# tongdaxu/VQ-VAE-from-Gaussian-VAE

Hardware: AMD Instinct MI355X
Metric: images/sec encode+quantize+decode, 256x256, codebook 2^16 (higher is better)
Workload: dtype f32

## Files before the change

### include/gqhip.h

```cpp
#ifndef GQHIP_H_
#define GQHIP_H_

#include <stdint.h>

#ifdef __cplusplus
extern "C" {
#endif

#define GQHIP_ABI_VERSION 8

typedef int64_t gqhip_gnstat_t;
#define GQHIP_GNSTAT_WORDS 8

typedef enum gqhip_status {
  GQHIP_OK = 0,
  GQHIP_ERR_INVALID_ARG = 1,
  GQHIP_ERR_WORKSPACE = 2,
  GQHIP_ERR_LAUNCH = 3,
  GQHIP_ERR_NO_DEVICE = 4
} gqhip_status;

int gqhip_abi_version(void);
const char *gqhip_status_string(int status);
int gqhip_last_hip_error(void);
// ... 73 lines not shown

int fsq_quantize_f32(const float *z, const int32_t *levels_host, int64_t nlev, float *zhat,
                     int32_t *idx, int64_t rows, void *stream);
int fsq_dequant_f32(const int32_t *idx, const int32_t *levels_host, int64_t nlev, float *zhat,
                    int64_t rows, void *stream);

#define GQHIP_LAYOUT_NCHW 0
#define GQHIP_LAYOUT_NHWC 1
int gn_silu_f32(const float *x, const float *gamma, const float *beta,
                const float *pre_bias_or_null, float *y, int64_t B, int64_t C, int64_t HW,
                int64_t groups, double eps, int apply_silu, int layout, gqhip_gnstat_t *stats_ws,
                void *stream);
int add_bias_f32(const float *a, const float *b, const float *bias_or_null, float *y, int64_t B,
                 int64_t C, int64_t HW, int layout, void *stream);

int add_bias_stats_f32(const float *a, const float *b, const float *bias_or_null, float *y, int64_t B,
                       int64_t C, int64_t HW, int64_t groups, gqhip_gnstat_t *stats_out, void *stream);

int gn_apply_f32(const float *x, const float *gamma, const float *beta, float *y, int64_t B, int64_t C,
                 int64_t HW, int64_t groups, double eps, int apply_silu, const gqhip_gnstat_t *stats, void *stream);

int gqhip_checksum_tensors(const void *table_dev, int64_t count, uint64_t *sums_dev, void *stream);

int gqhip_stats_prezeroed(int on);

int conv3x3_cin_small_f32(const float *x, const float *wk, const float *bias_or_null, float *y, int64_t *stats_out_or_null,
                          int64_t B, int64_t H, int64_t W, int64_t Cin, int64_t Cout, int64_t groups_out, void *stream);

int conv3x3_f32(const float *x, const float *gamma_or_null, const float *beta_or_null, const float *pre_bias_or_null,
                const gqhip_gnstat_t *stats_or_null, int64_t groups_in, double eps, int apply_silu, const float *wk,
                const float *bias_or_null, float *y, int64_t B, int64_t H, int64_t W, int64_t Cin, int64_t Cout, void *stream);

int upsample2x_nhwc_f32(const float *x, float *y, int64_t B, int64_t H, int64_t W, int64_t C,
                        void *stream);

int wino_in_nhwc_f32(const float *x, float *V, int64_t B, int64_t H, int64_t W, int64_t C, void *stream);
int wino_out_nhwc_f32(const float *M, float *y, int64_t B, int64_t H, int64_t W, int64_t C, float mscale, void *stream);

int wino_in_nhwc_f16x3(const float *x, void *V3, int64_t B, int64_t H, int64_t W, int64_t C, int tile, float scale,
                       void *stream);
int wino_in_nhwc_f16x2(const float *x, void *V2, int64_t B, int64_t H, int64_t W, int64_t C, int tile, float scale,
                       void *stream);
int wino_gemm_f16x2(const void *V2, const void *Wf, float *M, int64_t P, int64_t tiles, int64_t Cin, int64_t Cout,
                    void *stream);
int conv3x3_gn_f16x3(const float *x, const float *gamma, const float *beta, const float *pre_bias_or_null,
                     const gqhip_gnstat_t *stats_in, int64_t groups_in, double eps, int apply_silu, float scale, const void *Wf,
                     const float *bias_or_null, const float *res_or_null, float *y, gqhip_gnstat_t *stats_out_or_null, int64_t B,
                     int64_t H, int64_t W, int64_t Cin, int64_t Cout, int64_t groups_out, float mscale, void *stream);
int conv1x1_f16x3(const float *x, const float *pre_bias_or_null, const void *Wf, const float *scales_dev_or_null, float scale,
                  float mscale, const float *bias_or_null, const float *res_or_null, float *y, gqhip_gnstat_t *stats_out_or_null, int64_t B, int64_t HW,
                  int64_t Cin, int64_t Cout, int64_t groups_out, void *stream);
int conv1x1_gn_f16x3(const float *x, const float *gamma, const float *beta, const float *pre_bias_or_null,
                     const gqhip_gnstat_t *stats_in, int64_t groups_in, double eps, const void *Wf, float scale, float mscale,
                     const float *bias_or_null, const float *res_or_null, float *y, gqhip_gnstat_t *stats_out_or_null, int64_t B,
                     int64_t HW, int64_t Cin, int64_t Cout, int64_t groups_out, void *stream);
int conv1x1_qkv_split_f16x3(const float *x, const float *gamma_or_null, const float *beta_or_null, const float *pre_bias_or_null,
                            const gqhip_gnstat_t *stats_in_or_null, int64_t groups_in, double eps, const void *Wf, float scale,
                            float mscale, const float *bias_or_null, void *Q3, void *K3, void *V3, float sq, float sv, int64_t B,
                            int64_t L, int64_t C, void *stream);
int conv3x3s2_f16x3(const float *x, const void *Wf, const float *scales_dev_or_null, float scale, float mscale,
                    const float *bias_or_null, float *y, gqhip_gnstat_t *stats_out_or_null, int64_t B, int64_t Hin, int64_t Win,
                    int64_t Cin, int64_t Cout, int64_t groups_out, void *stream);
int upconv2x_f16x3(const float *x, const void *Wf, const float *scales_dev_or_null, float scale, float mscale,
                   const float *bias_or_null, float *y, gqhip_gnstat_t *stats_out_or_null, int64_t B, int64_t H, int64_t W,
                   int64_t Cin, int64_t Cout, int64_t groups_out, void *stream);
int conv3x3_gn_small_f32(const float *x, const float *gamma, const float *beta, const float *pre_bias_or_null,
                         const gqhip_gnstat_t *stats_in, int64_t groups_in, double eps, int apply_silu, const float *w_ohwi,
                         const float *bias_or_null, float *y, int64_t B, int64_t H, int64_t W, int64_t Cin, int64_t Cout,
                         void *stream);
int wino_in_gn_nhwc_f16x3(const float *x, const float *gamma, const float *beta, const float *pre_bias_or_null,
                          const gqhip_gnstat_t *stats, void *V3, int64_t B, int64_t H, int64_t W, int64_t C, int64_t groups,
                          double eps, int apply_silu, int tile, float scale, void *stream);
int wino_in_gn_nhwc_f16x2(const float *x, const float *gamma, const float *beta, const float *pre_bias_or_null,
                          const gqhip_gnstat_t *stats, void *V2, int64_t B, int64_t H, int64_t W, int64_t C, int64_t groups,
                          double eps, int apply_silu, int tile, float scale, void *stream);

int wino4_in_nhwc_f32(const float *x, float *V, int64_t B, int64_t H, int64_t W, int64_t C, void *stream);
int wino4_out_nhwc_f32(const float *M, float *y, int64_t B, int64_t H, int64_t W, int64_t C, float mscale, void *stream);

int wino_out_res_nhwc_f32(const float *M, const float *res, const float *bias_or_null, float *y, gqhip_gnstat_t *stats_out,
                          int64_t B, int64_t H, int64_t W, int64_t C, int64_t groups, int tile, float mscale,
                          void *stream);

int gn_stats_f32(const float *x, const float *pre_bias_or_null, int64_t B, int64_t C, int64_t HW, int64_t groups,
                 gqhip_gnstat_t *stats_out, void *stream);

int wino_in_gn_nhwc_f32(const float *x, const float *gamma, const float *beta, const float *pre_bias_or_null,
                        const gqhip_gnstat_t *stats, float *V, int64_t B, int64_t H, int64_t W, int64_t C,
                        int64_t groups, double eps, int apply_silu, void *stream);
int wino4_in_gn_nhwc_f32(const float *x, const float *gamma, const float *beta, const float *pre_bias_or_null,
                         const gqhip_gnstat_t *stats, float *V, int64_t B, int64_t H, int64_t W, int64_t C,
                         int64_t groups, double eps, int apply_silu, void *stream);

int attn_split_qkv_f16x3(const float *qkv, void *Q3, void *K3, void *V3, int64_t B, int64_t L, int64_t C, float sq, float sv,
                         void *stream);
int attn_softmax_split_f16x3(const float *S, void *P3, int64_t rows, int64_t L, float factor, void *stream);
int f16_scales_from_gn_stats(const gqhip_gnstat_t *stats, int64_t n_bg, double amp, double u_scale, float *scales_out,
                             void *stream);

int gq_index_histogram(const int64_t *idx, int64_t count, int64_t n,
                       int32_t *hist, void *stream);
int gq_indices_to_u16(const int64_t *idx, uint16_t *out, int64_t count,
                      void *stream);
int gq_indices_from_u16(const uint16_t *in, int64_t *idx, int64_t count,
                        void *stream);

int64_t gq_step_record_workspace_bytes(int64_t B, int64_t per_image);
int gq_step_record_f32(const float *x, const float *x_rec, const int64_t *idx, int32_t *rec, int64_t B, int64_t per_image,
                       int64_t n_idx, void *workspace_zeroed, int64_t workspace_bytes, void *stream);

int64_t gq_ssim_workspace_bytes(int64_t B, int64_t C, int64_t H, int64_t W);
int gq_ssim_f32(const float *x, const float *x_rec, int64_t B, int64_t C, int64_t H, int64_t W, int layout, int zero_mean,
                float *ssim_out_or_null, float *msssim_out_or_null, void *workspace_zeroed, int64_t workspace_bytes, void *stream);
int64_t gq_step_record_ssim_workspace_bytes(int64_t B, int64_t C, int64_t H, int64_t W);
int gq_step_record_ssim_f32(const float *x, const float *x_rec, const int64_t *idx, int32_t *rec, int64_t B, int64_t C, int64_t H,
                            int64_t W, int layout, int64_t n_idx, void *workspace_zeroed, int64_t workspace_bytes, void *stream);

int64_t gq_mha_workspace_bytes(int64_t B, int64_t L, int64_t E, int64_t H);
int gq_mha_fwd_f32(const float *qkv, float *out, int64_t B, int64_t L, int64_t E, int64_t H, void *workspace, void *stream);

int gqhip_profile_enable(int on);
int gqhip_profile_reserve(int pairs);
int gqhip_profile_collect(int *launches_host, double *total_ms_host);

int gqhip_debug_enable(int on);
int gqhip_debug_counters(const void *workspace, int64_t *fallback_rows_host,
                         int64_t *reranked_halftiles_host);
int gqhip_debug_grid(const void *workspace, const void *cb_cache_or_null, int64_t *out4_host);
#ifdef __cplusplus
}
#endif
#endif
```

### vq-vae-from-gaussian-vae_amd/csrc/gqhip_unet.hip

```cpp
#include "gqhip.h"

#include <hip/hip_ext.h>
#include <hip/hip_runtime.h>

#include <cstdlib>
#include <cstring>

#include "gqhip_internal.h"
#include "gq_unet_aux.h"
#include "gq_wino_gemm.h"
#include "gq_conv3.h"
#include "gq_conv_f32.h"
#include "gq_attn.h"

using namespace gqhip;

namespace {
thread_local int g_stats_prezeroed = 0;
inline hipError_t stats_zero(void *p, size_t bytes, hipStream_t st) {
  return g_stats_prezeroed ? hipSuccess : hipMemsetAsync(p, 0, bytes, st);
}
}

extern "C" {

int gqhip_stats_prezeroed(int on) {
  g_stats_prezeroed = on != 0;
  return GQHIP_OK;
}

int gn_silu_f32(const float *x, const float *gamma, const float *beta, const float *pre_bias_or_null, float *y,
                int64_t B, int64_t C, int64_t HW, int64_t groups, double eps, int apply_silu, int layout,
                int64_t *stats_ws, void *stream) {
  if (B < 0 || C < 1 || HW < 1 || groups < 1 || C % groups != 0) return GQHIP_ERR_INVALID_ARG;
  if (B == 0) return GQHIP_OK;
  if (!x || !gamma || !beta || !y || !stats_ws) return GQHIP_ERR_INVALID_ARG;
  hipStream_t st = static_cast<hipStream_t>(stream);
  const int64_t bg = B * groups, cpg = C / groups, chunk = cpg * HW;
  if (layout == GQHIP_LAYOUT_NHWC) {
    if (cpg % 4 != 0 || 256 % (C / 4) != 0 || groups > 64) return GQHIP_ERR_INVALID_ARG;
    if (stats_zero(stats_ws, sizeof(int64_t) * kStatWords * bg, st) != hipSuccess) return check_launch();
    const int lanes = (int)(256 / (C / 4));
    int slabs = (int)((HW + (int64_t)lanes * 16 - 1) / ((int64_t)lanes * 16));
    if (slabs > 1024) slabs = 1024;
    if (slabs < 1) slabs = 1;
    hipLaunchKernelGGL(gn_stats_nhwc_kernel, dim3((unsigned)(B * slabs)), dim3(256), 0, st, x, pre_bias_or_null,
                       stats_ws, (int)C, (long)HW, (int)cpg, slabs);
    int rc = check_launch();
    if (rc != GQHIP_OK) return rc;
    return launch(apply_silu ? gn_apply_nhwc_kernel<1> : gn_apply_nhwc_kernel<0>, dim3((unsigned)(B * slabs)), dim3(256), 0, st, x,
                  gamma, beta, y, stats_ws, pre_bias_or_null, (int)C, (long)HW, (int)cpg, eps, slabs);
  }
  if (layout != GQHIP_LAYOUT_NCHW || HW % 4 != 0) return GQHIP_ERR_INVALID_ARG;
  if (stats_zero(stats_ws, sizeof(int64_t) * kStatWords * bg, st) != hipSuccess) return check_launch();
  int slices = (int)((chunk + 4095) / 4096);
  if (slices > 256) slices = 256;
  if (slices < 1) slices = 1;
  hipLaunchKernelGGL(gn_stats_kernel, dim3((unsigned)(bg * slices)), dim3(256), 0, st, x, pre_bias_or_null, stats_ws,
                     (long)chunk, slices, (long)HW, (int)cpg, (int)groups);
  int rc = check_launch();
  if (rc != GQHIP_OK) return rc;
  int segs = (int)((HW + 8191) / 8192);
  if (segs < 1) segs = 1;
  const dim3 grid((unsigned)(B * C * segs));
  return launch(apply_silu ? gn_apply_kernel<1> : gn_apply_kernel<0>, grid, dim3(256), 0, st, x, gamma, beta, y, stats_ws,
                pre_bias_or_null, (int)C, (long)HW, (int)cpg, eps, segs);
}

int add_bias_f32(const float *a, const float *b, const float *bias_or_null, float *y, int64_t B, int64_t C,
                 int64_t HW, int layout, void *stream) {
  if (B < 0 || C < 1 || HW < 1) return GQHIP_ERR_INVALID_ARG;
  if (B == 0) return GQHIP_OK;
  if (!a || !b || !y) return GQHIP_ERR_INVALID_ARG;
  const long total4 = (long)(B * C * HW / 4);
  long blocks = (total4 + 255) / 256;
  if (blocks > 8192) blocks = 8192;
  hipStream_t st = static_cast<hipStream_t>(stream);
  if (layout == GQHIP_LAYOUT_NHWC) {
    if (C % 4 != 0) return GQHIP_ERR_INVALID_ARG;
    hipLaunchKernelGGL(add_bias_nhwc_kernel, dim3((unsigned)blocks), dim3(256), 0, st, a, b, bias_or_null, y, (int)C,
                       total4);
  } else {
    if (layout != GQHIP_LAYOUT_NCHW || HW % 4 != 0) return GQHIP_ERR_INVALID_ARG;
    hipLaunchKernelGGL(add_bias_kernel, dim3((unsigned)blocks), dim3(256), 0, st, a, b, bias_or_null, y, (int)C,
                       (long)HW, total4);
  }
  return check_launch();
}

static int nhwc_slabs(int64_t C, int64_t HW) {
  const int lanes = (int)(256 / (C / 4));
  int slabs = (int)((HW + (int64_t)lanes * 16 - 1) / ((int64_t)lanes * 16));
  if (slabs > 1024) slabs = 1024;
  return slabs < 1 ? 1 : slabs;
}

int add_bias_stats_f32(const float *a, const float *b, const float *bias_or_null, float *y, int64_t B, int64_t C,
                       int64_t HW, int64_t groups, int64_t *stats_out, void *stream) {
  if (B < 0 || C < 1 || HW < 1 || groups < 1 || C % groups != 0) return GQHIP_ERR_INVALID_ARG;
  if (B == 0) return GQHIP_OK;
  if (!a || !b || !y || !stats_out) return GQHIP_ERR_INVALID_ARG;
  const int64_t cpg = C / groups;
  if (cpg % 4 != 0 || 256 % (C / 4) != 0 || groups > 64) return GQHIP_ERR_INVALID_ARG;
  hipStream_t st = static_cast<hipStream_t>(stream);
// ... 444 lines not shown
  cp.H = (int)H; cp.W = (int)W; cp.Cin = (int)Cin; cp.Cout = (int)Cout; cp.cpg = gn ? (int)(Cin / groups_in) : 1; cp.eps = eps;
  const unsigned segs = (unsigned)(B * H * ((W + 31) / 32));
  if (Cin % 64 == 0) {
    const dim3 grid(segs, (unsigned)((Cout + 31) / 32));
    if (gn && apply_silu) hipLaunchKernelGGL((conv3x3_f32_ksplit_kernel<true, 1>), grid, dim3(256), 0, st, cp);
    else if (gn) hipLaunchKernelGGL((conv3x3_f32_ksplit_kernel<true, 0>), grid, dim3(256), 0, st, cp);
    else hipLaunchKernelGGL((conv3x3_f32_ksplit_kernel<false, 0>), grid, dim3(256), 0, st, cp);
    return check_launch();
  }
  if (gn) return GQHIP_ERR_INVALID_ARG;
  switch (Cin) {
    case 8: hipLaunchKernelGGL((conv3x3_f32_nsplit_kernel<8>), dim3(segs), dim3(256), 0, st, cp); break;
    case 16: hipLaunchKernelGGL((conv3x3_f32_nsplit_kernel<16>), dim3(segs), dim3(256), 0, st, cp); break;
    case 32: hipLaunchKernelGGL((conv3x3_f32_nsplit_kernel<32>), dim3(segs), dim3(256), 0, st, cp); break;
    default: return GQHIP_ERR_INVALID_ARG;
  }
  return check_launch();
}

int wino_out_nhwc_f32(const float *M, float *y, int64_t B, int64_t H, int64_t W, int64_t C, float mscale, void *stream) {
  if (B < 0 || H < 2 || W < 2 || H % 2 || W % 2 || C < 4 || C % 4 != 0) return GQHIP_ERR_INVALID_ARG;
  if (B == 0) return GQHIP_OK;
  if (!M || !y) return GQHIP_ERR_INVALID_ARG;
  const long tiles = (long)(B * (H / 2) * (W / 2)), total = tiles * (C / 4);
  long blocks = (total + 255) / 256;
  if (blocks > 16384) blocks = 16384;
  return launch(wino_out_nhwc_kernel, dim3((unsigned)blocks), dim3(256), 0, static_cast<hipStream_t>(stream), M, y,
                (int)H, (int)W, (int)(C / 4), tiles, total, mscale);
}

int wino4_in_nhwc_f32(const float *x, float *V, int64_t B, int64_t H, int64_t W, int64_t C, void *stream) {
  if (B < 0 || H < 4 || W < 4 || H % 4 || W % 4 || C < 4 || C % 4 != 0) return GQHIP_ERR_INVALID_ARG;
  if (B == 0) return GQHIP_OK;
  if (!x || !V) return GQHIP_ERR_INVALID_ARG;
  const long tiles = (long)(B * (H / 4) * (W / 4)), total = tiles * (C / 4);
  long blocks = (total + 255) / 256;
  if (blocks > 16384) blocks = 16384;
  return launch(wino4_in_nhwc_kernel<0>, dim3((unsigned)blocks), dim3(256), 0, static_cast<hipStream_t>(stream), x,
                (void *)V, (int)H, (int)W, (int)(C / 4), tiles, total, 1.0f);
}

int wino4_out_nhwc_f32(const float *M, float *y, int64_t B, int64_t H, int64_t W, int64_t C, float mscale, void *stream) {
  if (B < 0 || H < 4 || W < 4 || H % 4 || W % 4 || C < 4 || C % 4 != 0) return GQHIP_ERR_INVALID_ARG;
  if (B == 0) return GQHIP_OK;
  if (!M || !y) return GQHIP_ERR_INVALID_ARG;
  const long tiles = (long)(B * (H / 4) * (W / 4)), total = tiles * (C / 4);
  long blocks = (total + 255) / 256;
  if (blocks > 16384) blocks = 16384;
  return launch(wino4_out_nhwc_kernel, dim3((unsigned)blocks), dim3(256), 0, static_cast<hipStream_t>(stream), M, y,
                (int)H, (int)W, (int)(C / 4), tiles, total, mscale);
}

int wino_out_res_nhwc_f32(const float *M, const float *res, const float *bias_or_null, float *y, int64_t *stats_out,
                          int64_t B, int64_t H, int64_t W, int64_t C, int64_t groups, int tile, float mscale,
                          void *stream) {
  if ((tile != 2 && tile != 4) || B < 0 || H < tile || W < tile || H % tile || W % tile || C < 4 || C % 4 != 0 ||
      groups < 1 || C % groups != 0)
    return GQHIP_ERR_INVALID_ARG;
  if (B == 0) return GQHIP_OK;
  if (!M || !y || !stats_out) return GQHIP_ERR_INVALID_ARG;
  const int64_t cpg = C / groups;
  if (cpg % 4 != 0 || 256 % (C / 4) != 0 || groups > 64) return GQHIP_ERR_INVALID_ARG;
  hipStream_t st = static_cast<hipStream_t>(stream);
  if (stats_zero(stats_out, sizeof(int64_t) * kStatWords * B * groups, st) != hipSuccess) return check_launch();
  const long tpi = (long)((H / tile) * (W / tile)), tiles = (long)B * tpi;
  const int vw = (tile == 4 && 256 % (C / 2) == 0) ? 2 : 4;
  const int lanes = (int)(256 / (C / vw));
  long slabs = (tpi + (long)lanes * 4 - 1) / ((long)lanes * 4);
  if (slabs > 1024) slabs = 1024;
  if (slabs < 1) slabs = 1;
  const dim3 grid((unsigned)(B * slabs));
  if (tile == 4 && vw == 2)
    hipLaunchKernelGGL((wino_out_res_nhwc_kernel<4, 2>), grid, dim3(256), 0, st, M, res, bias_or_null, y, stats_out, (int)H,
                       (int)W, (int)(C / 2), (int)cpg, tiles, (int)slabs, mscale);
  else if (tile == 4)
    hipLaunchKernelGGL((wino_out_res_nhwc_kernel<4, 4>), grid, dim3(256), 0, st, M, res, bias_or_null, y, stats_out, (int)H,
                       (int)W, (int)(C / 4), (int)cpg, tiles, (int)slabs, mscale);
  else
    hipLaunchKernelGGL((wino_out_res_nhwc_kernel<2, 4>), grid, dim3(256), 0, st, M, res, bias_or_null, y, stats_out, (int)H,
                       (int)W, (int)(C / 4), (int)cpg, tiles, (int)slabs, mscale);
  return check_launch();
}

int attn_split_qkv_f16x3(const float *qkv, void *Q3, void *K3, void *V3, int64_t B, int64_t L, int64_t C, float sq, float sv,
                         void *stream) {
  if (B < 0 || L < 1 || C < 4 || C % 4 != 0 || !(sq > 0.f) || !(sv > 0.f)) return GQHIP_ERR_INVALID_ARG;
  if (B == 0) return GQHIP_OK;
  if (!qkv || !Q3 || !K3 || !V3) return GQHIP_ERR_INVALID_ARG;
  const long total = (long)(B * L * (C / 4));
  long blocks = (total + 255) / 256;
  if (blocks > 16384) blocks = 16384;
  return launch(attn_split_qkv_kernel, dim3((unsigned)blocks), dim3(256), 0, static_cast<hipStream_t>(stream), qkv,
                static_cast<_Float16 *>(Q3), static_cast<_Float16 *>(K3), static_cast<_Float16 *>(V3), (long)L,
                (int)(C / 4), sq, sv, total);
}

int attn_softmax_split_f16x3(const float *S, void *P3, int64_t rows, int64_t L, float factor, void *stream) {
  if (rows < 0 || L < 64 || L % 64 != 0 || L > 4096 || !(factor > 0.f)) return GQHIP_ERR_INVALID_ARG;
  if (rows == 0) return GQHIP_OK;
  if (!S || !P3) return GQHIP_ERR_INVALID_ARG;
  const dim3 grid((unsigned)((rows + 3) / 4));
  hipStream_t st = static_cast<hipStream_t>(stream);
  _Float16 *p = static_cast<_Float16 *>(P3);
#define GQ_SM(N) hipLaunchKernelGGL(attn_softmax_split_kernel<N>, grid, dim3(256), 0, st, S, p, (long)rows, factor)
  switch (L / 64) {
    case 1: GQ_SM(1); break;
    case 4: GQ_SM(4); break;
    case 16: GQ_SM(16); break;
    case 36: GQ_SM(36); break;
    case 64: GQ_SM(64); break;
    default: return GQHIP_ERR_INVALID_ARG;
  }
#undef GQ_SM
  return check_launch();
}

int f16_scales_from_gn_stats(const int64_t *stats, int64_t n_bg, double amp, double u_scale, float *scales_out,
                             void *stream) {
  if (!stats || !scales_out || n_bg < 1 || n_bg > 0x7fffffff || !(amp > 0.0) || !(u_scale > 0.0)) return GQHIP_ERR_INVALID_ARG;
  return launch(f16_scales_from_stats_kernel, dim3(1), dim3(64), 0, static_cast<hipStream_t>(stream), stats, (int)n_bg,
                (float)amp, (float)u_scale, scales_out);
}

int upsample2x_nhwc_f32(const float *x, float *y, int64_t B, int64_t H, int64_t W, int64_t C, void *stream) {
  if (B < 0 || H < 1 || W < 1 || C < 4 || C % 4 != 0) return GQHIP_ERR_INVALID_ARG;
  if (B == 0) return GQHIP_OK;
  if (!x || !y) return GQHIP_ERR_INVALID_ARG;
  const long total = (long)(B * H * W * (C / 4));
  long blocks = (total + 255) / 256;
  if (blocks > 16384) blocks = 16384;
  return launch(upsample2x_nhwc_kernel, dim3((unsigned)blocks), dim3(256), 0, static_cast<hipStream_t>(stream), x,
                y, (int)H, (int)W, (int)(C / 4), total);
}

int gqhip_checksum_tensors(const void *table_dev, int64_t count, uint64_t *sums_dev, void *stream) {
  if (count < 0 || count > 65535) return GQHIP_ERR_INVALID_ARG;
  if (count == 0) return GQHIP_OK;
  if (!table_dev || !sums_dev) return GQHIP_ERR_INVALID_ARG;
  hipStream_t st = static_cast<hipStream_t>(stream);
  if (hipMemsetAsync(sums_dev, 0, sizeof(uint64_t) * count, st) != hipSuccess) return check_launch();
  return launch(checksum_tensors_kernel, dim3((unsigned)count, kChecksumSlices), dim3(256), 0, st,
                static_cast<const ChecksumEntry *>(table_dev), reinterpret_cast<unsigned long long *>(sums_dev));
}

int64_t gq_mha_workspace_bytes(int64_t B, int64_t L, int64_t E, int64_t H) {
  (void)B; (void)L; (void)E; (void)H;
  return 0;
}

int gq_mha_fwd_f32(const float *qkv, float *out, int64_t B, int64_t L, int64_t E, int64_t H, void *workspace, void *stream) {
  (void)workspace;
  if (B < 0 || L < 0 || H < 1 || E != H * kAttnD || B * H > 65535 || L > (int64_t)0x7fffffff / 3 / E) return GQHIP_ERR_INVALID_ARG;
  if (B == 0 || L == 0) return GQHIP_OK;
  if (!qkv || !out || ((uintptr_t)qkv & 15) || ((uintptr_t)out & 15)) return GQHIP_ERR_INVALID_ARG;
  const dim3 grid((unsigned)((L + kAttnQRows - 1) / kAttnQRows), (unsigned)(B * H));
  return launch(mha_fwd_f32_kernel, grid, dim3(256), 0, static_cast<hipStream_t>(stream), qkv, out, (int)L, (int)E, (int)H);
}

}
```

### vq-vae-from-gaussian-vae_amd/pit_hip/_lib.py

```python
from __future__ import annotations

import ctypes
import threading
import math
import os
import subprocess
from typing import Optional, Tuple

import torch

_CSRC = os.path.normpath(os.path.join(os.path.dirname(os.path.abspath(__file__)), "..", "csrc"))
LIB_PATH = os.environ.get("GQHIP_LIB", os.path.join(_CSRC, "libgqhip.so"))

ABI_VERSION = 8
GNSTAT_WORDS = 8
GQHIP_LAYOUT = {"bchw": 0, "blc": 1}
GQHIP_GROUP_STRIDED = 0
GQHIP_GROUP_CONTIGUOUS = 1

_lib: Optional[ctypes.CDLL] = None

_vp = ctypes.c_void_p
_i64 = ctypes.c_int64
_SIGNATURES = {
    "gqhip_abi_version": (ctypes.c_int, []),
    "gqhip_status_string": (ctypes.c_char_p, [ctypes.c_int]),
    "gqhip_last_hip_error": (ctypes.c_int, []),
    "gqhip_workspace_bytes": (_i64, [_i64, _i64, _i64]),
    "gqhip_cb_cache_bytes": (_i64, [_i64, _i64]),
    "gqhip_grid_search_applies": (ctypes.c_int, [_i64, _i64]),
    "gqhip_cb_cache_degenerate": (ctypes.c_int, [_vp, _i64, _i64]),
    "gqhip_debug_grid": (ctypes.c_int, [_vp, _vp, ctypes.POINTER(_i64)]),
    "gqhip_set_filter": (ctypes.c_int, [ctypes.c_int]),
    "gqhip_get_filter": (ctypes.c_int, []),
    "gqhip_debug_plan": (ctypes.c_int, [_i64, _i64, _i64, ctypes.POINTER(_i64)]),
    "gq_scores_f32": (ctypes.c_int, [_vp, _vp, _vp, _vp, _i64, _i64, _i64, ctypes.c_double, _vp]),
    "gq_argmax_f32": (ctypes.c_int, [_vp, _vp, _vp, _vp, _vp, _vp, _i64, _i64, _i64, ctypes.c_double, _vp, _i64, _vp, _i64, _vp]),
    "gq_quantize_z_f32": (ctypes.c_int, [_vp, _vp, _vp, _vp, _vp, _vp, _vp, _vp, _i64, _i64, _i64, _i64, _i64,
                                         ctypes.c_int, ctypes.c_int, ctypes.c_double, ctypes.c_double,
                                         ctypes.c_double, _vp, _i64, _vp, _i64, _vp]),
    "gq_quantize_z_gauss_f32": (ctypes.c_int, [_vp, _vp, _vp, _vp, _vp, _vp, _vp, _vp, _vp, _vp, _i64, _i64, _i64, _i64, _i64,
                                               ctypes.c_int, ctypes.c_int, ctypes.c_double, ctypes.c_double, ctypes.c_double,
                                               ctypes.c_int, ctypes.c_double, ctypes.c_double, ctypes.c_double, ctypes.c_double,
                                               ctypes.c_double, ctypes.c_int, _vp, _i64, _vp, _i64, _vp]),
    "gq_gauss_train_f32": (ctypes.c_int, [_vp, _vp, _vp, _vp, _vp, _vp, _vp, _i64, _i64, _i64, _i64, ctypes.c_int, ctypes.c_int,
                                          ctypes.c_double, ctypes.c_double, ctypes.c_double, ctypes.c_double, ctypes.c_double,
                                          ctypes.c_double, ctypes.c_double, ctypes.c_int, ctypes.c_double, _vp]),
    "gq_gauss_backward_f32": (ctypes.c_int, [_vp, _vp, _vp, _vp, _vp, _vp, _vp, _i64, _i64, _i64, _i64, ctypes.c_int, ctypes.c_int,
                                             ctypes.c_double, ctypes.c_double, ctypes.c_double, ctypes.c_double, ctypes.c_double,
                                             _vp]),
    "vq_quantize_z_f32": (ctypes.c_int, [_vp, _vp, _vp, _vp, _vp, _i64, _i64, _i64, _i64, _i64, ctypes.c_int, ctypes.c_double,
                                         ctypes.c_int, _vp, _i64, _vp, _i64, _vp]),
    "gq_dequant_f32": (ctypes.c_int, [_vp, _vp, _vp, _i64, _i64, _i64, _i64, _i64, ctypes.c_int,
                                      ctypes.c_int, _vp]),
    "vq_argmin_f32": (ctypes.c_int, [_vp, _vp, _vp, _vp, _i64, _i64, _i64, _vp, _i64, _vp, _i64, _vp]),
    "lfq_pack_f32": (ctypes.c_int, [_vp, _vp, _vp, _i64, _i64, _vp]),
    "lfq_unpack_f32": (ctypes.c_int, [_vp, _vp, _i64, _i64, _vp]),
    "fsq_quantize_f32": (ctypes.c_int, [_vp, ctypes.POINTER(ctypes.c_int32), _i64, _vp, _vp, _i64, _vp]),
    "fsq_dequant_f32": (ctypes.c_int, [_vp, ctypes.POINTER(ctypes.c_int32), _i64, _vp, _i64, _vp]),
    "gn_silu_f32": (ctypes.c_int, [_vp, _vp, _vp, _vp, _vp, _i64, _i64, _i64, _i64, ctypes.c_double, ctypes.c_int,
                                   ctypes.c_int, _vp, _vp]),
    "add_bias_stats_f32": (ctypes.c_int, [_vp, _vp, _vp, _vp, _i64, _i64, _i64, _i64, _vp, _vp]),
    "gn_apply_f32": (ctypes.c_int, [_vp, _vp, _vp, _vp, _i64, _i64, _i64, _i64, ctypes.c_double, ctypes.c_int, _vp, _vp]),
    "wino_in_nhwc_f32": (ctypes.c_int, [_vp, _vp, _i64, _i64, _i64, _i64, _vp]),
    "wino4_in_nhwc_f32": (ctypes.c_int, [_vp, _vp, _i64, _i64, _i64, _i64, _vp]),
    "wino4_out_nhwc_f32": (ctypes.c_int, [_vp, _vp, _i64, _i64, _i64, _i64, ctypes.c_float, _vp]),
    "wino_out_res_nhwc_f32": (ctypes.c_int, [_vp, _vp, _vp, _vp, _vp, _i64, _i64, _i64, _i64, _i64, ctypes.c_int,
                                              ctypes.c_float, _vp]),
    "wino_in_nhwc_f16x3": (ctypes.c_int, [_vp, _vp, _i64, _i64, _i64, _i64, ctypes.c_int, ctypes.c_float, _vp]),
    "wino_in_nhwc_f16x2": (ctypes.c_int, [_vp, _vp, _i64, _i64, _i64, _i64, ctypes.c_int, ctypes.c_float, _vp]),
    "wino_gemm_f16x2": (ctypes.c_int, [_vp, _vp, _vp, _i64, _i64, _i64, _i64, _vp]),
    "upconv2x_f16x3": (ctypes.c_int, [_vp, _vp, _vp, ctypes.c_float, ctypes.c_float, _vp, _vp, _vp, _i64, _i64, _i64, _i64, _i64, _i64,
                                      _vp]),
    "attn_split_qkv_f16x3": (ctypes.c_int, [_vp, _vp, _vp, _vp, _i64, _i64, _i64, ctypes.c_float, ctypes.c_float, _vp]),
    "attn_softmax_split_f16x3": (ctypes.c_int, [_vp, _vp, _i64, _i64, ctypes.c_float, _vp]),
    "wino_in_gn_nhwc_f16x3": (ctypes.c_int, [_vp, _vp, _vp, _vp, _vp, _vp, _i64, _i64, _i64, _i64, _i64, ctypes.c_double,
                                              ctypes.c_int, ctypes.c_int, ctypes.c_float, _vp]),
    "wino_in_gn_nhwc_f16x2": (ctypes.c_int, [_vp, _vp, _vp, _vp, _vp, _vp, _i64, _i64, _i64, _i64, _i64, ctypes.c_double,
                                              ctypes.c_int, ctypes.c_int, ctypes.c_float, _vp]),
    "conv3x3_gn_f16x3": (ctypes.c_int, [_vp, _vp, _vp, _vp, _vp, _i64, ctypes.c_double, ctypes.c_int, ctypes.c_float, _vp,
                                         _vp, _vp, _vp, _vp, _i64, _i64, _i64, _i64, _i64, _i64, ctypes.c_float, _vp]),
    "conv1x1_f16x3": (ctypes.c_int, [_vp, _vp, _vp, _vp, ctypes.c_float, ctypes.c_float, _vp, _vp, _vp, _vp, _i64, _i64, _i64, _i64, _i64,
                                      _vp]),
    "conv1x1_gn_f16x3": (ctypes.c_int, [_vp, _vp, _vp, _vp, _vp, _i64, ctypes.c_double, _vp, ctypes.c_float, ctypes.c_float, _vp, _vp,
                                         _vp, _vp, _i64, _i64, _i64, _i64, _i64, _vp]),
    "conv1x1_qkv_split_f16x3": (ctypes.c_int, [_vp, _vp, _vp, _vp, _vp, _i64, ctypes.c_double, _vp, ctypes.c_float, ctypes.c_float,
                                                _vp, _vp, _vp, _vp, ctypes.c_float, ctypes.c_float, _i64, _i64, _i64, _vp]),
    "conv3x3s2_f16x3": (ctypes.c_int, [_vp, _vp, _vp, ctypes.c_float, ctypes.c_float, _vp, _vp, _vp, _i64, _i64, _i64, _i64, _i64,
                                        _i64, _vp]),
    "conv3x3_gn_small_f32": (ctypes.c_int, [_vp, _vp, _vp, _vp, _vp, _i64, ctypes.c_double, ctypes.c_int, _vp, _vp, _vp, _i64, _i64,
                                             _i64, _i64, _i64, _vp]),
    "conv3x3_cin_small_f32": (ctypes.c_int, [_vp, _vp, _vp, _vp, _vp, _i64, _i64, _i64, _i64, _i64, _i64, _vp]),
    "conv3x3_f32": (ctypes.c_int, [_vp, _vp, _vp, _vp, _vp, _i64, ctypes.c_double, ctypes.c_int, _vp, _vp, _vp, _i64, _i64, _i64,
                                   _i64, _i64, _vp]),
    "gqhip_checksum_tensors": (ctypes.c_int, [_vp, _i64, _vp, _vp]),
    "gn_stats_f32": (ctypes.c_int, [_vp, _vp, _i64, _i64, _i64, _i64, _vp, _vp]),
    "wino_in_gn_nhwc_f32": (ctypes.c_int, [_vp, _vp, _vp, _vp, _vp, _vp, _i64, _i64, _i64, _i64, _i64, ctypes.c_double,
                                            ctypes.c_int, _vp]),
    "wino4_in_gn_nhwc_f32": (ctypes.c_int, [_vp, _vp, _vp, _vp, _vp, _vp, _i64, _i64, _i64, _i64, _i64, ctypes.c_double,
                                             ctypes.c_int, _vp]),
    "wino_out_nhwc_f32": (ctypes.c_int, [_vp, _vp, _i64, _i64, _i64, _i64, ctypes.c_float, _vp]),
    "f16_scales_from_gn_stats": (ctypes.c_int, [_vp, _i64, ctypes.c_double, ctypes.c_double, _vp, _vp]),
    "upsample2x_nhwc_f32": (ctypes.c_int, [_vp, _vp, _i64, _i64, _i64, _i64, _vp]),
    "add_bias_f32": (ctypes.c_int, [_vp, _vp, _vp, _vp, _i64, _i64, _i64, ctypes.c_int, _vp]),
    "gqhip_stats_prezeroed": (ctypes.c_int, [ctypes.c_int]),
    "gq_index_histogram": (ctypes.c_int, [_vp, _i64, _i64, _vp, _vp]),
    "gq_indices_to_u16": (ctypes.c_int, [_vp, _vp, _i64, _vp]),
    "gq_indices_from_u16": (ctypes.c_int, [_vp, _vp, _i64, _vp]),
    "gq_step_record_workspace_bytes": (_i64, [_i64, _i64]),
    "gq_step_record_f32": (ctypes.c_int, [_vp, _vp, _vp, _vp, _i64, _i64, _i64, _vp, _i64, _vp]),
    "gq_ssim_workspace_bytes": (_i64, [_i64, _i64, _i64, _i64]),
    "gq_ssim_f32": (ctypes.c_int, [_vp, _vp, _i64, _i64, _i64, _i64, ctypes.c_int, ctypes.c_int, _vp, _vp, _vp, _i64, _vp]),
    "gq_step_record_ssim_workspace_bytes": (_i64, [_i64, _i64, _i64, _i64]),
    "gq_step_record_ssim_f32": (ctypes.c_int, [_vp, _vp, _vp, _vp, _i64, _i64, _i64, _i64, ctypes.c_int, _i64, _vp, _i64, _vp]),
    "gq_mha_workspace_bytes": (_i64, [_i64, _i64, _i64, _i64]),
    "gq_mha_fwd_f32": (ctypes.c_int, [_vp, _vp, _i64, _i64, _i64, _i64, _vp, _vp]),
    "gqhip_profile_enable": (ctypes.c_int, [ctypes.c_int]),
    "gqhip_profile_reserve": (ctypes.c_int, [ctypes.c_int]),
    "gqhip_profile_collect": (ctypes.c_int, [ctypes.POINTER(ctypes.c_int), ctypes.POINTER(ctypes.c_double)]),
    "gqhip_debug_enable": (ctypes.c_int, [ctypes.c_int]),
    "gqhip_debug_counters": (ctypes.c_int, [_vp, ctypes.POINTER(_i64), ctypes.POINTER(_i64)]),
}
EXPORTED_SYMBOLS = tuple(_SIGNATURES)


class GqHipError(RuntimeError):
    pass


def build(force: bool = False) -> str:
    args = ["make", "-C", _CSRC, "-s", "-j4"]
    if force:
        args.append("-B")
    subprocess.check_call(args + ["libgqhip.so"])
    return LIB_PATH


def lib() -> ctypes.CDLL:
    global _lib
    if _lib is None:
        if not os.path.exists(LIB_PATH):
            raise GqHipError(
                f"{LIB_PATH} is missing: run `python -c 'import __graft_entry__ as g; g.build()'` "
                "(or `make -C vq-vae-from-gaussian-vae_amd/csrc`). There is no CPU fallback."
            )
        L = ctypes.CDLL(LIB_PATH)
        for name, (res, args) in _SIGNATURES.items():
            fn = getattr(L, name)
            fn.restype = res
            fn.argtypes = args
        if L.gqhip_abi_version() != ABI_VERSION:
            raise GqHipError("libgqhip.so ABI version mismatch")
        _lib = L
    return _lib


def _check(rc: int, what: str) -> None:
    if rc != 0:
        L = lib()
        raise GqHipError(f"{what}: {L.gqhip_status_string(rc).decode()} (hipError {L.gqhip_last_hip_error()})")


def _dev(t: torch.Tensor, dtype: torch.dtype, name: str) -> torch.Tensor:
    if not isinstance(t, torch.Tensor) or not t.is_cuda:
        raise GqHipError(f"{name} must be a tensor on a HIP device (got {getattr(t, 'device', type(t))}); "
                         "the HIP path has no CPU fallback")
    if t.dtype != dtype:
        raise GqHipError(f"{name} must be {dtype}, got {t.dtype}")
    return t if t.is_contiguous() else t.contiguous()


def _stream() -> int:
    return torch.cuda.current_stream().cuda_stream


def _ptr(t: Optional[torch.Tensor]) -> Optional[int]:
    return None if t is None else t.data_ptr()


class Workspace:

    def __init__(self) -> None:
        self.buf: Optional[torch.Tensor] = None
        self.cache_buf: Optional[torch.Tensor] = None
# ... 289 lines not shown


def fsq_dequant(idx, levels):
    idx = _dev(idx, torch.int32, "indices")
    arr, n = _levels(levels)
    rows = idx.numel()
    zhat = torch.empty(rows, n, dtype=torch.float32, device=idx.device)
    with torch.cuda.device(idx.device):
        _check(lib().fsq_dequant_f32(idx.data_ptr(), arr, n, zhat.data_ptr(), rows, _stream()), "fsq_dequant_f32")
    return zhat


def image_layout(x: torch.Tensor):
    if x.dim() != 4:
        return None
    if x.is_contiguous():
        return 0
    if x.is_contiguous(memory_format=torch.channels_last):
        return 1
    return None


class StatsArena:

    def __init__(self) -> None:
        self.buf, self.used, self.want = None, 0, 0

    def begin(self, device) -> None:
        if self.buf is None or self.buf.device != device or self.buf.numel() < self.want:
            self.buf = torch.zeros(max(self.want, 1), dtype=torch.int64, device=device)
        elif self.used:
            self.buf[: self.used].zero_()
        self.used = self.want = 0

    def take(self, nwords: int):
        self.want += nwords
        if self.buf is None or self.used + nwords > self.buf.numel():
            return None
        t = self.buf[self.used: self.used + nwords]
        self.used += nwords
        return t


class _ArenaState(threading.local):
    def __init__(self) -> None:
        self.state = {"active": None, "flag": 0}


_ARENA_TLS = _ArenaState()


class stats_arena:

    def __init__(self, arena: StatsArena, device) -> None:
        self.arena, self.device = arena, device

    def __enter__(self):
        self.prev = _ARENA_TLS.state["active"]
        self.arena.begin(self.device)
        _ARENA_TLS.state["active"] = self.arena
        return self.arena

    def __exit__(self, *exc):
        _ARENA_TLS.state["active"] = self.prev
        _set_prezeroed(0)


def _set_prezeroed(on: int) -> None:
    if _ARENA_TLS.state["flag"] != on:
        lib().gqhip_stats_prezeroed(on)
        _ARENA_TLS.state["flag"] = on


def _stats_records(nwords: int, device):
    a = _ARENA_TLS.state["active"]
    t = a.take(nwords) if a is not None else None
    if t is not None and t.device == device:
        _set_prezeroed(1)
        return t
    _set_prezeroed(0)
    return torch.empty(nwords, dtype=torch.int64, device=device)


def gn_nhwc_ok(C: int, groups: int) -> bool:
    cpg = C // groups
    return C % groups == 0 and cpg % 4 == 0 and C % 4 == 0 and 256 % (C // 4) == 0 and groups <= 64


def gn_silu(x, gamma, beta, groups: int, eps: float, silu: bool = True, pre_bias=None):
    layout = image_layout(x)
    if not x.is_cuda or x.dtype != torch.float32 or layout is None:
        raise GqHipError("gn_silu needs a dense fp32 NCHW / channels_last HIP tensor")
    B, C = x.shape[0], x.shape[1]
    HW = x.shape[2] * x.shape[3]
    ws = _stats_records(GNSTAT_WORDS * B * groups, x.device)
    y = torch.empty_like(x)
    with torch.cuda.device(x.device):
        _check(lib().gn_silu_f32(x.data_ptr(), gamma.data_ptr(), beta.data_ptr(), _ptr(pre_bias), y.data_ptr(), B, C, HW,
                                 groups, float(eps), 1 if silu else 0, layout, ws.data_ptr(), _stream()), "gn_silu_f32")
    return y


def add_bias(a, b, bias=None):
    layout = image_layout(a)
    if layout is None or image_layout(b) != layout or not a.is_cuda or a.dtype != torch.float32:
        raise GqHipError("add_bias needs two dense fp32 HIP tensors of the same layout")
    B, C = a.shape[0], a.shape[1]
    HW = a.shape[2] * a.shape[3]
    y = torch.empty_like(a)
    with torch.cuda.device(a.device):
        _check(lib().add_bias_f32(a.data_ptr(), b.data_ptr(), _ptr(bias), y.data_ptr(), B, C, HW, layout, _stream()),
               "add_bias_f32")
    return y


def add_bias_stats(a, b, bias, groups: int):
    if image_layout(a) != 1 or image_layout(b) != 1 or not a.is_cuda or a.dtype != torch.float32 or not gn_nhwc_ok(a.shape[1], groups):
        raise GqHipError("add_bias_stats needs two dense channels_last fp32 HIP tensors with a GroupNorm-compatible C")
    B, C = a.shape[0], a.shape[1]
    HW = a.shape[2] * a.shape[3]
    y = torch.empty_like(a)
    stats = _stats_records(GNSTAT_WORDS * B * groups, a.device)
    with torch.cuda.device(a.device):
        _check(lib().add_bias_stats_f32(a.data_ptr(), b.data_ptr(), _ptr(bias), y.data_ptr(), B, C, HW, groups,
                                        stats.data_ptr(), _stream()), "add_bias_stats_f32")
    return y, stats


def gn_apply(x, gamma, beta, groups: int, eps: float, silu: bool, stats):
    if image_layout(x) != 1 or not x.is_cuda or x.dtype != torch.float32:
        raise GqHipError("gn_apply needs a dense channels_last fp32 HIP tensor")
    B, C = x.shape[0], x.shape[1]
    HW = x.shape[2] * x.shape[3]
    y = torch.empty_like(x)
    with torch.cuda.device(x.device):
        _check(lib().gn_apply_f32(x.data_ptr(), gamma.data_ptr(), beta.data_ptr(), y.data_ptr(), B, C, HW, groups,
                                  float(eps), 1 if silu else 0, stats.data_ptr(), _stream()), "gn_apply_f32")
    return y


def gn_stats_values(stats):
    r = stats.view(-1, GNSTAT_WORDS).double()
    s = (r[:, 2] * 2.0 ** 24 + r[:, 1] * 2.0 ** -16) + r[:, 0] * 2.0 ** -56
    ss = (r[:, 5] * 2.0 ** 24 + r[:, 4] * 2.0 ** -16) + r[:, 3] * 2.0 ** -56
    bad = r[:, 6] != 0
    s = torch.where(bad, torch.full_like(s, float("nan")), s)
    ss = torch.where(bad, torch.full_like(ss, float("nan")), ss)
    return torch.stack([s, ss], 1).flatten()


def gn_stats(x, groups: int, pre_bias=None):
    if image_layout(x) != 1 or not x.is_cuda or x.dtype != torch.float32 or not gn_nhwc_ok(x.shape[1], groups):
        raise GqHipError("gn_stats needs a dense channels_last fp32 HIP tensor with a GroupNorm-compatible C")
    B, C = x.shape[0], x.shape[1]
    stats = _stats_records(GNSTAT_WORDS * B * groups, x.device)
    with torch.cuda.device(x.device):
        _check(lib().gn_stats_f32(x.data_ptr(), _ptr(pre_bias), B, C, x.shape[2] * x.shape[3], groups, stats.data_ptr(),
                                  _stream()), "gn_stats_f32")
    return stats


def wino_conv3x3(x, U, gn=None, residual=None, bias=None, stats_groups: int = 0, f16=None):
    if image_layout(x) != 1 or not x.is_cuda or x.dtype != torch.float32 or x.shape[1] % 4 or x.shape[2] % 2 or x.shape[3] % 2:
        raise GqHipError("wino_conv3x3 needs a dense channels_last fp32 HIP tensor, C % 4 == 0, even H and W")
    B, C, H, W = x.shape
    cout = U.shape[2]
    f4 = U.shape[0] == 36
    if f4 and (H % 4 or W % 4):
        raise GqHipError("F(4x4,3x3) needs H, W multiples of 4")
    t = 4 if f4 else 2
    tiles = B * (H // t) * (W // t)
    L = lib()
    mscale = 1.0
    with torch.cuda.device(x.device):
        if f16 is not None:
            U3, u_scale, x_bound = f16[:3]
            amp = 100.0 if f4 else 4.0
            v_scale = 2.0 ** math.floor(math.log2(32768.0 / (amp * max(float(x_bound), 1e-30))))
            v_scale = min(v_scale, 2.0 ** 14)
            use_own = len(f16) > 3 and f16[3] is not None and tiles % 256 == 0 and own_gemm_fits(U.shape[0], tiles, cout, C)
            if use_own:
                V = torch.empty((U.shape[0], tiles, 2 * C), dtype=torch.float16, device=x.device)
                if gn is not None:
                    gamma, beta, groups, eps, silu, stats, pre_bias = gn
                    _check(L.wino_in_gn_nhwc_f16x2(x.data_ptr(), gamma.data_ptr(), beta.data_ptr(), _ptr(pre_bias),
                                                   stats.data_ptr(), V.data_ptr(), B, H, W, C, groups, float(eps),
                                                   1 if silu else 0, t, float(v_scale), _stream()), "wino_in_gn_nhwc_f16x2")
                else:
                    _check(L.wino_in_nhwc_f16x2(x.data_ptr(), V.data_ptr(), B, H, W, C, t, float(v_scale), _stream()),
                           "wino_in_nhwc_f16x2")
                M = torch.empty((U.shape[0], tiles, cout), dtype=torch.float32, device=x.device)
                _check(L.wino_gemm_f16x2(V.data_ptr(), f16[3].data_ptr(), M.data_ptr(), U.shape[0], tiles, C, cout,
                                         _stream()), "wino_gemm_f16x2")
                V = None
            else:
                V = torch.empty((U.shape[0], tiles, 3 * C), dtype=torch.float16, device=x.device)
            if V is None:
                pass
            elif gn is not None:
                gamma, beta, groups, eps, silu, stats, pre_bias = gn
                _check(L.wino_in_gn_nhwc_f16x3(x.data_ptr(), gamma.data_ptr(), beta.data_ptr(), _ptr(pre_bias),
                                               stats.data_ptr(), V.data_ptr(), B, H, W, C, groups, float(eps),
                                               1 if silu else 0, t, float(v_scale), _stream()), "wino_in_gn_nhwc_f16x3")
            else:
                _check(L.wino_in_nhwc_f16x3(x.data_ptr(), V.data_ptr(), B, H, W, C, t, float(v_scale), _stream()),
                       "wino_in_nhwc_f16x3")
            if V is not None:
                M = torch.bmm(V, U3, out_dtype=torch.float32)
            mscale = 1.0 / (v_scale * u_scale)
        else:
            V = torch.empty((U.shape[0], tiles, C), dtype=x.dtype, device=x.device)
            if gn is not None:
                gamma, beta, groups, eps, silu, stats, pre_bias = gn
                _check((L.wino4_in_gn_nhwc_f32 if f4 else L.wino_in_gn_nhwc_f32)(
                    x.data_ptr(), gamma.data_ptr(), beta.data_ptr(), _ptr(pre_bias), stats.data_ptr(), V.data_ptr(), B, H, W, C,
                    groups, float(eps), 1 if silu else 0, _stream()), "wino_in_gn_nhwc_f32")
            else:
                _check((L.wino4_in_nhwc_f32 if f4 else L.wino_in_nhwc_f32)(x.data_ptr(), V.data_ptr(), B, H, W, C, _stream()),
                       "wino_in_nhwc_f32")
            M = torch.bmm(V, U)
        y = torch.empty((B, cout, H, W), dtype=x.dtype, device=x.device, memory_format=torch.channels_last)
        if stats_groups:
            if (residual is not None and (image_layout(residual) != 1 or tuple(residual.shape) != tuple(y.shape))) \
                    or not gn_nhwc_ok(cout, stats_groups):
                raise GqHipError("fused Winograd tail needs a channels_last residual of the output shape and a GroupNorm-compatible C")
            stats = _stats_records(GNSTAT_WORDS * B * stats_groups, x.device)
            _check(L.wino_out_res_nhwc_f32(M.data_ptr(), _ptr(residual), _ptr(bias), y.data_ptr(), stats.data_ptr(),
                                           B, H, W, cout, stats_groups, t, float(mscale), _stream()), "wino_out_res_nhwc_f32")
            return y, stats
        _check((L.wino4_out_nhwc_f32 if f4 else L.wino_out_nhwc_f32)(M.data_ptr(), y.data_ptr(), B, H, W, cout,
                                                                     float(mscale), _stream()), "wino_out_nhwc_f32")
    return y


_BMM_OUT_DTYPE = None


def bmm_out_dtype_ok(device) -> bool:
    global _BMM_OUT_DTYPE
    if _BMM_OUT_DTYPE is None:
        try:
            a = torch.ones(1, 16, 16, dtype=torch.float16, device=device)
            _BMM_OUT_DTYPE = bool(torch.bmm(a, a, out_dtype=torch.float32).dtype == torch.float32)
        except (TypeError, RuntimeError):
            _BMM_OUT_DTYPE = False
    return _BMM_OUT_DTYPE


ATTN_L_OK = (64, 256, 1024, 2304, 4096)


def attention_scales(q_bound: float, v_bound: float):
    pow2 = lambda bound: min(2.0 ** math.floor(math.log2(32768.0 / max(float(bound), 1e-30))), 2.0 ** 14)
    return pow2(q_bound), pow2(v_bound)


def attention_operands(B: int, Ltok: int, C: int, device):
    return (torch.empty((B, Ltok, 3 * C), dtype=torch.float16, device=device),
            torch.empty((B, Ltok, 3 * C), dtype=torch.float16, device=device),
            torch.empty((B, 3 * Ltok, C), dtype=torch.float16, device=device))


def attention_from_operands(Q3, K3, V3, sq: float, sv: float):
    B, Ltok, C3 = Q3.shape
    C = C3 // 3
    if Ltok not in ATTN_L_OK:
        raise GqHipError("attention_f16x3: token count %d not in %s" % (Ltok, ATTN_L_OK))
    L_ = lib()
    with torch.cuda.device(Q3.device):
        S = torch.bmm(Q3, K3.transpose(1, 2), out_dtype=torch.float32)
        P3 = torch.empty((B, Ltok, 3 * Ltok), dtype=torch.float16, device=Q3.device)
        _check(L_.attn_softmax_split_f16x3(S.data_ptr(), P3.data_ptr(), B * Ltok, Ltok, float(C) ** -0.5 / (sq * sq), _stream()),
               "attn_softmax_split_f16x3")
        O = torch.bmm(P3, V3, out_dtype=torch.float32)
    return O, 1.0 / (16384.0 * sv)


def attention_f16x3(qkv, q_bound: float, v_bound: float):
    if not (qkv.is_cuda and qkv.dtype == torch.float32 and qkv.dim() == 3 and qkv.is_contiguous() and qkv.shape[2] % 12 == 0):
        raise GqHipError("attention_f16x3 needs a dense fp32 HIP tensor [B, L, 3C], C % 4 == 0")
    B, Ltok, C3 = qkv.shape
    C = C3 // 3
    if Ltok not in ATTN_L_OK:
        raise GqHipError("attention_f16x3: token count %d not in %s" % (Ltok, ATTN_L_OK))
    sq, sv = attention_scales(q_bound, v_bound)
    with torch.cuda.device(qkv.device):
        Q3, K3, V3 = attention_operands(B, Ltok, C, qkv.device)
        _check(lib().attn_split_qkv_f16x3(qkv.data_ptr(), Q3.data_ptr(), K3.data_ptr(), V3.data_ptr(), B, Ltok, C, sq, sv,
                                          _stream()), "attn_split_qkv_f16x3")
    return attention_from_operands(Q3, K3, V3, sq, sv)

# ... 472 lines not shown
```

Measured before the change: 494.7.

## Add fused Winograd conv3x3 entry with cached workspace and batch slabbing

```diff
diff --git a/include/gqhip.h b/include/gqhip.h
--- a/include/gqhip.h
+++ b/include/gqhip.h
@@ -179,6 +179,15 @@
                           int64_t B, int64_t H, int64_t W, int64_t C, int64_t groups, int tile, float mscale,
                           void *stream);
 
+int wino_conv3x3_f16x2(const float *x, const float *gamma_or_null, const float *beta, const float *pre_bias_or_null,
+                       const gqhip_gnstat_t *stats_in, int64_t groups_in, double eps, int apply_silu, const void *Wf,
+                       const float *bias_or_null, const float *res_or_null, float *y, gqhip_gnstat_t *stats_out,
+                       int64_t groups_out, int64_t B, int64_t H, int64_t W, int64_t Cin, int64_t Cout, int tile, float v_scale,
+                       float mscale, void *workspace, int64_t workspace_bytes, int64_t slab, void *stream);
+int64_t gqhip_wino_workspace_bytes(int64_t P, int64_t slab_tiles, int64_t Cin, int64_t Cout);
+int64_t gqhip_wino_slab_plan(int64_t P, int64_t tiles_per_image, int64_t B, int64_t Cin, int64_t Cout);
+int64_t gqhip_wino_slab_pick(int64_t P, int64_t tiles_per_image, int64_t B, int64_t Cin, int64_t Cout);
+
 int gn_stats_f32(const float *x, const float *pre_bias_or_null, int64_t B, int64_t C, int64_t HW, int64_t groups,
                  gqhip_gnstat_t *stats_out, void *stream);
 
diff --git a/vq-vae-from-gaussian-vae_amd/csrc/gqhip_unet.hip b/vq-vae-from-gaussian-vae_amd/csrc/gqhip_unet.hip
--- a/vq-vae-from-gaussian-vae_amd/csrc/gqhip_unet.hip
+++ b/vq-vae-from-gaussian-vae_amd/csrc/gqhip_unet.hip
@@ -20,6 +20,9 @@
 inline hipError_t stats_zero(void *p, size_t bytes, hipStream_t st) {
   return g_stats_prezeroed ? hipSuccess : hipMemsetAsync(p, 0, bytes, st);
 }
+
+constexpr int64_t kWinoSlabBudgetBytes = 0;
+constexpr double kWinoSlabFill = 0.85;
 }
 
 extern "C" {
@@ -630,6 +633,79 @@
   return check_launch();
 }
 
+int64_t gqhip_wino_workspace_bytes(int64_t P, int64_t slab_tiles, int64_t Cin, int64_t Cout) {
+  if (P < 1 || slab_tiles < 0 || Cin < 1 || Cout < 1 || P > 36 || Cin > 4096 || Cout > 4096 || slab_tiles > 0x3fffffff) return -1;
+  return P * slab_tiles * (4 * Cin + 4 * Cout);
+}
+
+static bool wino_slab_valid(int64_t tpi, int64_t B, int64_t slab) {
+  return slab >= 1 && slab <= B && (slab * tpi) % 256 == 0 && ((B % slab) * tpi) % 256 == 0;
+}
+
+int64_t gqhip_wino_slab_plan(int64_t P, int64_t tiles_per_image, int64_t B, int64_t Cin, int64_t Cout) {
+  if (P < 1 || tiles_per_image < 1 || B < 1 || Cin < 1 || Cout < 1) return 0;
+  const int64_t per_image = gqhip_wino_workspace_bytes(P, tiles_per_image, Cin, Cout);
+  if (per_image <= 0 || kWinoSlabBudgetBytes <= 0 || per_image * B <= kWinoSlabBudgetBytes) return B;
+  const int64_t cols = (Cin % 64 == 0 && Cout % 256 == 0) ? 256 : 128, rows = cols == 256 ? 128 : 256;
+  for (int64_t s = kWinoSlabBudgetBytes / per_image < B ? kWinoSlabBudgetBytes / per_image : B; s >= 1; --s) {
+    if (!wino_slab_valid(tiles_per_image, B, s)) continue;
+    const double rounds = (double)P * (double)(s * tiles_per_image / rows) * (double)(Cout / cols) / 512.0;
+    const double whole = rounds == (double)(int64_t)rounds ? rounds : (double)((int64_t)rounds + 1);
+    if (rounds >= 1.0 && rounds / whole >= kWinoSlabFill) return s;
+  }
+  return B;
+}
+
+int64_t gqhip_wino_slab_pick(int64_t P, int64_t tiles_per_image, int64_t B, int64_t Cin, int64_t Cout) {
+  if (B < 1 || tiles_per_image < 1) return 0;
+  int64_t slab = gqhip_wino_slab_plan(P, tiles_per_image, B, Cin, Cout);
+  if (const char *knob = getenv("GQHIP_WINO_SLAB")) {
+    char *end = nullptr;
+    const long long v = strtoll(knob, &end, 10);
+    if (end != knob && *end == '\0' && v >= 0) slab = v == 0 || v > B ? B : (int64_t)v;
+  }
+  return wino_slab_valid(tiles_per_image, B, slab) ? slab : B;
+}
+
+int wino_conv3x3_f16x2(const float *x, const float *gamma_or_null, const float *beta, const float *pre_bias_or_null,
+                       const int64_t *stats_in, int64_t groups_in, double eps, int apply_silu, const void *Wf,
+                       const float *bias_or_null, const float *res_or_null, float *y, int64_t *stats_out, int64_t groups_out,
+                       int64_t B, int64_t H, int64_t W, int64_t Cin, int64_t Cout, int tile, float v_scale, float mscale,
+                       void *workspace, int64_t workspace_bytes, int64_t slab, void *stream) {
+  if ((tile != 2 && tile != 4) || B < 0 || H < tile || W < tile || H % tile || W % tile || Cin < 32 || Cin > 4096 || Cout < 128 ||
+      Cout > 4096 || groups_out < 0 || (gamma_or_null && groups_in < 1))
+    return GQHIP_ERR_INVALID_ARG;
+  if (B == 0) return GQHIP_OK;
+  if (!x || !Wf || !y || !workspace || (gamma_or_null && (!beta || !stats_in)) || (groups_out > 0 && !stats_out))
+    return GQHIP_ERR_INVALID_ARG;
+  if (groups_out == 0 && (bias_or_null || res_or_null)) return GQHIP_ERR_INVALID_ARG;
+  const int64_t P = tile == 4 ? 36 : 16, tpi = (H / tile) * (W / tile);
+  if (!wino_slab_valid(tpi, B, slab)) slab = B;
+  if ((B * tpi) % 256 != 0 || Cin % 32 != 0 || Cout % 128 != 0) return GQHIP_ERR_INVALID_ARG;
+  const int64_t need = gqhip_wino_workspace_bytes(P, slab * tpi, Cin, Cout);
+  if (need < 0 || workspace_bytes < need) return GQHIP_ERR_INVALID_ARG;
+  const int64_t pix_in = H * W * Cin, pix_out = H * W * Cout;
+  for (int64_t b0 = 0; b0 < B; b0 += slab) {
+    const int64_t nb = B - b0 < slab ? B - b0 : slab, tiles = nb * tpi;
+    void *V = workspace;
+    float *M = reinterpret_cast<float *>(static_cast<char *>(workspace) + P * tiles * 4 * Cin);
+    int rc = gamma_or_null
+                 ? wino_in_gn_nhwc_f16x2(x + b0 * pix_in, gamma_or_null, beta, pre_bias_or_null, stats_in + kStatWords * b0 * groups_in,
+                                         V, nb, H, W, Cin, groups_in, eps, apply_silu, tile, v_scale, stream)
+                 : wino_in_nhwc_f16x2(x + b0 * pix_in, V, nb, H, W, Cin, tile, v_scale, stream);
+    if (rc != GQHIP_OK) return rc;
+    rc = wino_gemm_f16x2(V, Wf, M, P, tiles, Cin, Cout, stream);
+    if (rc != GQHIP_OK) return rc;
+    if (groups_out > 0)
+      rc = wino_out_res_nhwc_f32(M, res_or_null ? res_or_null + b0 * pix_out : nullptr, bias_or_null, y + b0 * pix_out,
+                                 stats_out + kStatWords * b0 * groups_out, nb, H, W, Cout, groups_out, tile, mscale, stream);
+    else
+      rc = (tile == 4 ? wino4_out_nhwc_f32 : wino_out_nhwc_f32)(M, y + b0 * pix_out, nb, H, W, Cout, mscale, stream);
+    if (rc != GQHIP_OK) return rc;
+  }
+  return GQHIP_OK;
+}
+
 int attn_split_qkv_f16x3(const float *qkv, void *Q3, void *K3, void *V3, int64_t B, int64_t L, int64_t C, float sq, float sv,
                          void *stream) {
   if (B < 0 || L < 1 || C < 4 || C % 4 != 0 || !(sq > 0.f) || !(sv > 0.f)) return GQHIP_ERR_INVALID_ARG;
diff --git a/vq-vae-from-gaussian-vae_amd/pit_hip/_lib.py b/vq-vae-from-gaussian-vae_amd/pit_hip/_lib.py
--- a/vq-vae-from-gaussian-vae_amd/pit_hip/_lib.py
+++ b/vq-vae-from-gaussian-vae_amd/pit_hip/_lib.py
@@ -100,6 +100,12 @@
     "wino4_in_gn_nhwc_f32": (ctypes.c_int, [_vp, _vp, _vp, _vp, _vp, _vp, _i64, _i64, _i64, _i64, _i64, ctypes.c_double,
                                              ctypes.c_int, _vp]),
     "wino_out_nhwc_f32": (ctypes.c_int, [_vp, _vp, _i64, _i64, _i64, _i64, ctypes.c_float, _vp]),
+    "wino_conv3x3_f16x2": (ctypes.c_int, [_vp, _vp, _vp, _vp, _vp, _i64, ctypes.c_double, ctypes.c_int, _vp, _vp, _vp, _vp, _vp,
+                                           _i64, _i64, _i64, _i64, _i64, _i64, ctypes.c_int, ctypes.c_float, ctypes.c_float,
+                                           _vp, _i64, _i64, _vp]),
+    "gqhip_wino_workspace_bytes": (_i64, [_i64, _i64, _i64, _i64]),
+    "gqhip_wino_slab_plan": (_i64, [_i64, _i64, _i64, _i64, _i64]),
+    "gqhip_wino_slab_pick": (_i64, [_i64, _i64, _i64, _i64, _i64]),
     "f16_scales_from_gn_stats": (ctypes.c_int, [_vp, _i64, ctypes.c_double, ctypes.c_double, _vp, _vp]),
     "upsample2x_nhwc_f32": (ctypes.c_int, [_vp, _vp, _i64, _i64, _i64, _i64, _vp]),
     "add_bias_f32": (ctypes.c_int, [_vp, _vp, _vp, _vp, _i64, _i64, _i64, ctypes.c_int, _vp]),
@@ -555,6 +561,23 @@
     return torch.empty(nwords, dtype=torch.int64, device=device)
 
 
+_WINO_WS = {}
+
+
+def _wino_workspace(nbytes: int, device):
+    if nbytes < 0:
+        raise GqHipError("wino_conv3x3: shape out of range for the Winograd workspace")
+    if torch.cuda.is_current_stream_capturing():
+        return torch.empty(max(nbytes, 1), dtype=torch.uint8, device=device)
+    key = (device.index if device.index is not None else torch.cuda.current_device(), _stream())
+    buf = _WINO_WS.get(key)
+    if buf is None or buf.numel() < nbytes:
+        _WINO_WS.pop(key, None)
+        buf = None
+        buf = _WINO_WS[key] = torch.empty(max(nbytes, 1), dtype=torch.uint8, device=device)
+    return buf
+
+
 def gn_nhwc_ok(C: int, groups: int) -> bool:
     cpg = C // groups
     return C % groups == 0 and cpg % 4 == 0 and C % 4 == 0 and 256 % (C // 4) == 0 and groups <= 64
@@ -653,24 +676,24 @@
             v_scale = min(v_scale, 2.0 ** 14)
             use_own = len(f16) > 3 and f16[3] is not None and tiles % 256 == 0 and own_gemm_fits(U.shape[0], tiles, cout, C)
             if use_own:
-                V = torch.empty((U.shape[0], tiles, 2 * C), dtype=torch.float16, device=x.device)
-                if gn is not None:
-                    gamma, beta, groups, eps, silu, stats, pre_bias = gn
-                    _check(L.wino_in_gn_nhwc_f16x2(x.data_ptr(), gamma.data_ptr(), beta.data_ptr(), _ptr(pre_bias),
-                                                   stats.data_ptr(), V.data_ptr(), B, H, W, C, groups, float(eps),
-                                                   1 if silu else 0, t, float(v_scale), _stream()), "wino_in_gn_nhwc_f16x2")
-                else:
-                    _check(L.wino_in_nhwc_f16x2(x.data_ptr(), V.data_ptr(), B, H, W, C, t, float(v_scale), _stream()),
-                           "wino_in_nhwc_f16x2")
-                M = torch.empty((U.shape[0], tiles, cout), dtype=torch.float32, device=x.device)
-                _check(L.wino_gemm_f16x2(V.data_ptr(), f16[3].data_ptr(), M.data_ptr(), U.shape[0], tiles, C, cout,
-                                         _stream()), "wino_gemm_f16x2")
-                V = None
-            else:
-                V = torch.empty((U.shape[0], tiles, 3 * C), dtype=torch.float16, device=x.device)
-            if V is None:
-                pass
-            elif gn is not None:
+                if stats_groups and ((residual is not None and (image_layout(residual) != 1 or tuple(residual.shape) != (B, cout, H, W)))
+                                     or not gn_nhwc_ok(cout, stats_groups)):
+                    raise GqHipError("fused Winograd tail needs a channels_last residual of the output shape and a GroupNorm-compatible C")
+                P, tpi = U.shape[0], tiles // B
+                slab = L.gqhip_wino_slab_pick(P, tpi, B, C, cout)
+                ws = _wino_workspace(L.gqhip_wino_workspace_bytes(P, slab * tpi, C, cout), x.device)
+                y = torch.empty((B, cout, H, W), dtype=x.dtype, device=x.device, memory_format=torch.channels_last)
+                ostats = _stats_records(GNSTAT_WORDS * B * stats_groups, x.device) if stats_groups else None
+                gamma, beta, groups, eps, silu, stats, pre_bias = gn if gn is not None else (None, None, 0, 0.0, False, None, None)
+                _check(L.wino_conv3x3_f16x2(x.data_ptr(), _ptr(gamma), _ptr(beta), _ptr(pre_bias), _ptr(stats), groups, float(eps),
+                                            1 if silu else 0, f16[3].data_ptr(), _ptr(bias) if stats_groups else None,
+                                            _ptr(residual) if stats_groups else None, y.data_ptr(),
+                                            _ptr(ostats), stats_groups, B, H, W, C, cout, t, float(v_scale),
+                                            1.0 / (v_scale * u_scale), ws.data_ptr(), ws.numel(), slab, _stream()),
+                       "wino_conv3x3_f16x2")
+                return (y, ostats) if stats_groups else y
+            V = torch.empty((U.shape[0], tiles, 3 * C), dtype=torch.float16, device=x.device)
+            if gn is not None:
                 gamma, beta, groups, eps, silu, stats, pre_bias = gn
                 _check(L.wino_in_gn_nhwc_f16x3(x.data_ptr(), gamma.data_ptr(), beta.data_ptr(), _ptr(pre_bias),
                                                stats.data_ptr(), V.data_ptr(), B, H, W, C, groups, float(eps),
@@ -678,8 +701,7 @@
             else:
                 _check(L.wino_in_nhwc_f16x3(x.data_ptr(), V.data_ptr(), B, H, W, C, t, float(v_scale), _stream()),
                        "wino_in_nhwc_f16x3")
-            if V is not None:
-                M = torch.bmm(V, U3, out_dtype=torch.float32)
+            M = torch.bmm(V, U3, out_dtype=torch.float32)
             mscale = 1.0 / (v_scale * u_scale)
         else:
             V = torch.empty((U.shape[0], tiles, C), dtype=x.dtype, device=x.device)
```

Result: no change. 493.6 (-0.2%).
